# zhaoyuhsin/Edge-Guided-Near-Eye-Image-Analysis-for-Head-Mounted-Displays

Measured on AMD Instinct MI355X. Metric: eye-frames/sec (320x240): inference edge+seg (value), +fit, exact fp32, and train fwd+bwd at 1 MI355X, higher is better.
Workload: dtype f32 tensors; inference products split into f16 hi/lo pairs (3 f16 MFMAs per product, 22-bit significand), f32 accumulate (`exact_fp32`: every product on the f32 MFMA); `train`: bf16 storage, f32 accumulate, f32 master weights (and an f32-storage leg)

## Files before the change

edge-guided-near-eye-image-analysis-for-head-mounted-displays_amd/csrc/common.h:

```cpp
#pragma once
#include <hip/hip_runtime.h>
#include <cstdarg>
#include <cstdio>
#include <mutex>
#include <unordered_map>
#include "../../include/egne_hip.h"

static __device__ __attribute__((aligned(256), used)) float egne_zero_page[64] = {0};

typedef __bf16 egne_bf16;
typedef float egne_f32x4 __attribute__((ext_vector_type(4)));
typedef __bf16 egne_bf16x4 __attribute__((ext_vector_type(4)));
typedef __bf16 egne_bf16x8 __attribute__((ext_vector_type(8)));

__device__ __forceinline__ egne_f32x4 ld4(const float* p) { return *(const egne_f32x4*)p; }
__device__ __forceinline__ egne_f32x4 ld4(const egne_bf16* p) { return __builtin_convertvector(*(const egne_bf16x4*)p, egne_f32x4); }
__device__ __forceinline__ void st4(float* p, egne_f32x4 v) { *(egne_f32x4*)p = v; }
__device__ __forceinline__ void st4(egne_bf16* p, egne_f32x4 v) { *(egne_bf16x4*)p = __builtin_convertvector(v, egne_bf16x4); }
__device__ __forceinline__ float ld1(const float* p) { return *p; }
__device__ __forceinline__ float ld1(const egne_bf16* p) { return (float)*p; }
__device__ __forceinline__ void st1(float* p, float v) { *p = v; }
__device__ __forceinline__ void st1(egne_bf16* p, float v) { *p = (egne_bf16)v; }
template <typename T> struct egne_vt { static constexpr int N = 4; };
template <> struct egne_vt<egne_bf16> { static constexpr int N = 8; };
template <int N> struct egne_fv { float v[N]; };
__device__ __forceinline__ egne_fv<4> ldv(const float* p) {
  const egne_f32x4 t = *(const egne_f32x4*)p;
  return egne_fv<4>{{t[0], t[1], t[2], t[3]}};
}
__device__ __forceinline__ egne_fv<8> ldv(const egne_bf16* p) {
  typedef unsigned u4_ __attribute__((ext_vector_type(4)));
  const u4_ w = *(const u4_*)p;
  egne_fv<8> r;
#pragma unroll
  for (int i = 0; i < 4; ++i) {
    r.v[2 * i] = __builtin_bit_cast(float, w[i] << 16);
    r.v[2 * i + 1] = __builtin_bit_cast(float, w[i] & 0xffff0000u);
  }
  return r;
}
__device__ __forceinline__ void stv(float* p, const egne_fv<4>& a) { *(egne_f32x4*)p = egne_f32x4{a.v[0], a.v[1], a.v[2], a.v[3]}; }
__device__ __forceinline__ void stv(egne_bf16* p, const egne_fv<8>& a) {
  const egne_f32x4 lo = {a.v[0], a.v[1], a.v[2], a.v[3]}, hi = {a.v[4], a.v[5], a.v[6], a.v[7]};
  const egne_bf16x4 l = __builtin_convertvector(lo, egne_bf16x4), h = __builtin_convertvector(hi, egne_bf16x4);
  *(egne_bf16x8*)p = egne_bf16x8{l[0], l[1], l[2], l[3], h[0], h[1], h[2], h[3]};
}
typedef unsigned egne_u32x4 __attribute__((ext_vector_type(4)));
template <typename T> __device__ __forceinline__ egne_u32x4 ldraw(const T* p) { return *(const egne_u32x4*)p; }
__device__ __forceinline__ egne_fv<4> unpackv(const float*, egne_u32x4 w) {
  return egne_fv<4>{{__builtin_bit_cast(float, w[0]), __builtin_bit_cast(float, w[1]), __builtin_bit_cast(float, w[2]), __builtin_bit_cast(float, w[3])}};
}
__device__ __forceinline__ egne_fv<8> unpackv(const egne_bf16*, egne_u32x4 w) {
  egne_fv<8> r;
#pragma unroll
  for (int i = 0; i < 4; ++i) {
    r.v[2 * i] = __builtin_bit_cast(float, w[i] << 16);
    r.v[2 * i + 1] = __builtin_bit_cast(float, w[i] & 0xffff0000u);
  }
  return r;
}
template <int N> __device__ __forceinline__ egne_fv<N> ldf(const float* p) {
  egne_fv<N> r;
#pragma unroll
  for (int i = 0; i < N; i += 4) { const egne_f32x4 t = *(const egne_f32x4*)(p + i); r.v[i] = t[0]; r.v[i + 1] = t[1]; r.v[i + 2] = t[2]; r.v[i + 3] = t[3]; }
  return r;
}
template <int N> __device__ __forceinline__ egne_fv<N> fv_fill(float x) {
  egne_fv<N> r;
#pragma unroll
  for (int i = 0; i < N; ++i) r.v[i] = x;
  return r;
}
template <typename T> __device__ __forceinline__ const T* zero_page() { return (const T*)egne_zero_page; }

#ifdef EGNE_NO_OVF_CHECK
__device__ __forceinline__ bool egne_nonfinite(float) { return false; }
__device__ __forceinline__ bool egne_nonfinite64(double) { return false; }
#else
__device__ __forceinline__ bool egne_nonfinite(float v) { return __builtin_amdgcn_classf(v, 0x207); }
__device__ __forceinline__ bool egne_nonfinite64(double v) { return !__builtin_isfinite(v); }
#endif
__device__ __forceinline__ bool egne_ovf_row(int y, int H) { return y % 3 == 1 || y == H - 1; }
__device__ __forceinline__ void egne_ovf_commit(bool bad, unsigned* flag) {
  if (flag && bad) atomicOr(flag, 1u);
}

namespace egne {

char* err_buf();

inline int fail(int code, const char* fmt, ...) {
  va_list ap;
  va_start(ap, fmt);
  vsnprintf(err_buf(), 512, fmt, ap);
  va_end(ap);
  return code;
}

inline bool fp32_storage(const egne_conv_desc& d) {
  for (int i = 0; i < d.nseg && i < EGNE_MAXSEG; ++i)
    if (d.seg[i].presplit != 0) return false;
  return d.out_split == 0;
}

inline int check_launch(const char* what) {
  hipError_t e = hipGetLastError();
  if (e != hipSuccess) return fail(EGNE_ERR_LAUNCH, "%s: %s", what, hipGetErrorString(e));
  return EGNE_OK;
}

inline bool raise_lds(const void* kern, size_t bytes) {
  static std::mutex mu;
  static std::unordered_map<const void*, size_t> have;
  std::lock_guard<std::mutex> g(mu);
  auto it = have.find(kern);
  if (it != have.end() && it->second >= bytes) return true;
  if (hipFuncSetAttribute(kern, hipFuncAttributeMaxDynamicSharedMemorySize, (int)bytes) != hipSuccess) {
    (void)hipGetLastError();
    return false;
  }
  have[kern] = bytes;
  return true;
}
template <typename... K> inline bool raise_lds_all(size_t bytes, K... kern) { return (raise_lds((const void*)kern, bytes) && ...); }

#define EGNE_REQUIRE(cond, ...) \
  do { if (!(cond)) return ::egne::fail(EGNE_ERR_ARG, __VA_ARGS__); } while (0)

bool halo3_supported(const egne_conv_desc& d);
int halo3_launch(const egne_conv_desc& d, hipStream_t st);

bool wgrad_halo_supported(const egne_conv_desc& d, long long gzs);
int wgrad_halo_splits(const egne_conv_desc& d);
int wgrad_halo_launch(const egne_conv_desc& d, const float* gz, long long gzs, int gzo, float* ws, hipStream_t st);
int wgrad_halo_f16_launch(const egne_conv_desc& d, const float* gz, long long gzs, int gzo, const unsigned* gz_dyn, float* ws, hipStream_t st);

bool wgrad3x3_bf16_supported(const egne_conv_desc& d, long long gzs);
int wgrad3x3_bf16_splits(const egne_conv_desc& d);
int wgrad3x3_bf16_launch(const egne_conv_desc& d, const egne_bf16* gz, long long gzs, int gzo, float* ws, hipStream_t st);
bool wgrad1x1_bf16_supported(const egne_conv_desc& d, long long gzs);
int wgrad1x1_bf16_splits(const egne_conv_desc& d);
int wgrad1x1_bf16_launch(const egne_conv_desc& d, const egne_bf16* gz, long long gzs, int gzo, float* ws, hipStream_t st);

inline int cdiv(long long a, long long b) { return (int)((a + b - 1) / b); }

}
```

edge-guided-near-eye-image-analysis-for-head-mounted-displays_amd/csrc/conv_halo_f16.hip:

```cpp
#include "common.h"
#include "kernel_util.h"
#include "split_f16.h"

namespace {

constexpr int KC = 32, LDH = 40, TW = 32;

__device__ __forceinline__ float act1(float v, int act) {
  if (act == EGNE_ACT_RELU) return fmaxf(v, 0.f);
  if (act == EGNE_ACT_LEAKY) return v > 0.f ? v : 0.01f * v;
  return v;
}


template <int WM, int WN, int D, bool LAT, int NW, int PF = 0, bool TP = false, bool POOL = false, int NP = 3, bool PS = false>
__global__ __launch_bounds__(256, 2) void conv3x3_halo_f16_kernel(const egne_conv_desc p, const _Float16* __restrict__ fhi,
                                                               const _Float16* __restrict__ flo, float a_scale,
                                                               float out_scale, int tiles_x, int tiles_y, int ntiles) {
  egne::dyn_scales(p.dyn_scale, a_scale, out_scale);
  const int vH = TP ? p.W : p.H, vW = TP ? p.H : p.W, rstep = TP ? 1 : p.W, cstep = TP ? p.W : 1;
  constexpr int TH = (4 / NW) * WM;
  constexpr int d = D;
  constexpr int HWd = TW + 2 * d, HHd = TH + 2 * d, npx = HHd * HWd;
  constexpr int nitems = npx * 8;
  constexpr int NI = (nitems + 255) / 256;
  static_assert(HWd >= 32, "one wrap per 32-pixel step");
  static_assert(WN < 3 || (NP == 3 && !PS && !POOL && !LAT && NW == 1), "96-wide tile: three products, fp32 slices, no pooled output");
  extern __shared__ __attribute__((aligned(16))) _Float16 ldsh[];
  _Float16* Ahi = ldsh;
  _Float16* Alo = ldsh + npx * LDH;

  const int tid = threadIdx.x, lane = tid & 63, wave = tid >> 6;
  const int li = lane & 31, lh = lane >> 5;
  const int wrow = wave / NW;
  const int nt0 = (blockIdx.y * NW + wave % NW) * WN;
  const int NT = p.CoutP >> 5, KT16 = p.Ktot >> 4;
  const egne_seg sg = p.seg[0];
  const int Cp = sg.Cp;
  const int c4 = tid & 7;
  const int wave_s = __builtin_amdgcn_readfirstlane(wave);
  auto fresh_tid = [&]() {
    int l;
    asm volatile("v_mbcnt_lo_u32_b32 %0, -1, 0\n\tv_mbcnt_hi_u32_b32 %0, -1, %0" : "=v"(l));
    return wave_s * 64 + l;
  };
  const int S = LAT ? p.dil[0] : 1;
  const unsigned frame_in = (unsigned)p.H * p.W * (unsigned)sg.pix_stride * 4u;
  const unsigned frame_out = (unsigned)p.H * p.W * (unsigned)p.out_pix_stride * 4u;
  const unsigned frame_res = (unsigned)p.H * p.W * (unsigned)p.res_pix_stride * 4u;

  constexpr bool LEAN = WN >= 3;
  int hyx[LEAN ? 1 : NI], roff[LEAN ? 1 : NI];
  if constexpr (!LEAN) {
    int px = tid >> 3;
    int hy = px / HWd, hx = px - hy * HWd;
#pragma unroll
    for (int i = 0; i < NI; ++i) {
      const bool in = tid + 256 * i < nitems;
      hyx[i] = in ? ((S * hy) << 16) | (S * hx) : 0x7fff7fff;
      roff[i] = (S * hy * rstep + S * hx * cstep) * (int)sg.pix_stride * 4 + (PS ? (c4 >> 2) * 64 + (c4 & 3) * 16 : c4 * 16);
      hx += 32;
      if (hx >= HWd) { hx -= HWd; ++hy; }
    }
  }
  const int lofs0 = (tid >> 3) * LDH + c4 * 4;

  struct Tile { int b, y0, x0, py, px; };
  auto tile_of = [&](int t) {
    Tile r;
    const int tx = t % tiles_x; t /= tiles_x;
    const int ty = t % tiles_y; t /= tiles_y;
    r.py = 0; r.px = 0;
    if (LAT) { r.px = t % S; t /= S; r.py = t % S; t /= S; }
    r.b = t; r.y0 = ty * TH; r.x0 = tx * TW;
    return r;
  };

  unsigned goff[NI];
  __amdgpu_buffer_rsrc_t rin = make_rsrc(sg.ptr, 0);
  int stage_b = 0;
  auto map_tile = [&](const Tile& tl) {
    const int ybase = tl.py + S * (tl.y0 - d), xbase = tl.px + S * (tl.x0 - d);
    const int tbase = ((ybase * rstep + xbase * cstep) * (int)sg.pix_stride + sg.ch_off) * 4;
    if constexpr (LEAN) {
      const int tf = fresh_tid();
      const int px = tf >> 3, c4f = tf & 7;
      int hy = px / HWd, hx = px - hy * HWd;
#pragma unroll
      for (int i = 0; i < NI; ++i) {
        const unsigned iy = (unsigned)(ybase + S * hy), ix = (unsigned)(xbase + S * hx);
        const bool in = tf + 256 * i < nitems && iy < (unsigned)vH && ix < (unsigned)vW;
        goff[i] = in ? (unsigned)(tbase + (S * hy * rstep + S * hx * cstep) * (int)sg.pix_stride * 4 + c4f * 16) : OOB;
        hx += 32;
        if (hx >= HWd) { hx -= HWd; ++hy; }
      }
    } else {
#pragma unroll
    for (int i = 0; i < NI; ++i) {
      const unsigned iy = (unsigned)(ybase + (hyx[i] >> 16)), ix = (unsigned)(xbase + (hyx[i] & 0xffff));
      goff[i] = (iy < (unsigned)vH && ix < (unsigned)vW) ? (unsigned)(tbase + roff[i]) : OOB;
    }
    }
    rin = make_rsrc(sg.ptr + (long long)tl.b * p.H * p.W * sg.pix_stride, frame_in);
    stage_b = tl.b;
  };

  u32x4 st[NI];
  f32x4 st_sc = {1.f, 1.f, 1.f, 1.f}, st_sh = {0.f, 0.f, 0.f, 0.f};
  unsigned st_cmask = 0;
  int st_c0 = 0;
  auto load_affine = [&]() {
    const int cq = (LEAN ? fresh_tid() & 7 : c4) * 4;
    const bool cok = st_c0 + cq < Cp;
    st_sc = *(const f32x4*)(cok ? sg.scale + (long long)stage_b * Cp + st_c0 + cq : egne_zero_page);
    st_sh = *(const f32x4*)(cok ? sg.shift + (long long)stage_b * Cp + st_c0 + cq : egne_zero_page);
  };
  auto load_chunk = [&](int c0) {
    const bool cok = PS || c0 + (LEAN ? fresh_tid() & 7 : c4) * 4 < Cp;
    st_cmask = cok ? 0u : OOB;
    st_c0 = c0;
    if (!LEAN && sg.scale) load_affine();
#pragma unroll
    for (int i = 0; i < NI; ++i) st[i] = __builtin_amdgcn_raw_buffer_load_b128(rin, (int)(goff[i] | st_cmask), c0 * 4, 0);
  };
  const float slope_in = sg.act_in == EGNE_ACT_RELU ? 0.f : (sg.act_in == EGNE_ACT_LEAKY ? 0.01f : 1.f);
  const float slope_out = p.act == EGNE_ACT_RELU ? 0.f : (p.act == EGNE_ACT_LEAKY ? 0.01f : 1.f);
  auto store_chunk = [&]() {
    if (sg.scale) {
#pragma unroll
      for (int i = 0; i < NI; ++i) {
        f32x4 v = __builtin_bit_cast(f32x4, st[i]) * st_sc + st_sh;
#pragma unroll
        for (int e = 0; e < 4; ++e) v[e] = fmaxf(v[e], v[e] * slope_in);
        if ((goff[i] | st_cmask) & OOB) v = (f32x4)(0.f);
        st[i] = __builtin_bit_cast(u32x4, v);
      }
    }
    const int tid_s = LEAN ? fresh_tid() : tid;
    const int lofs_s = LEAN ? (tid_s >> 3) * LDH + (tid_s & 7) * 4 : lofs0;
#pragma unroll
    for (int i = 0; i < NI; ++i) {
      if (i < NI - 1 || tid_s + 256 * i < nitems) {
        const f32x4 v = __builtin_bit_cast(f32x4, st[i]);
        const int o = lofs_s + i * 32 * LDH;
        if constexpr (PS) {
          *(u32x4*)&(c4 >> 2 ? Alo : Ahi)[(tid >> 3) * LDH + (c4 & 3) * 8 + i * 32 * LDH] = st[i];
          continue;
        }
        if constexpr (NP == 1) {
          float t0, t1, t2, t3;
          asm("v_mul_f32_e32 %0, %1, %2" : "=v"(t0) : "s"(a_scale), "v"(v[0]));
          asm("v_mul_f32_e32 %0, %1, %2" : "=v"(t1) : "s"(a_scale), "v"(v[1]));
          asm("v_mul_f32_e32 %0, %1, %2" : "=v"(t2) : "s"(a_scale), "v"(v[2]));
          asm("v_mul_f32_e32 %0, %1, %2" : "=v"(t3) : "s"(a_scale), "v"(v[3]));
          const egne::sp_f32x2 u0 = {t0, t1}, u1 = {t2, t3};
          const h2 h0 = __builtin_convertvector(u0, h2), h1 = __builtin_convertvector(u1, h2);
          const h4 hi = {h0[0], h0[1], h1[0], h1[1]};
          *(h4*)&Ahi[o] = hi;
          continue;
        }
        h2 h0, h1, l0, l1;
        egne::split2(v[0], v[1], a_scale, h0, l0);
        egne::split2(v[2], v[3], a_scale, h1, l1);
        const h4 hi = {h0[0], h0[1], h1[0], h1[1]}, lo = {l0[0], l0[1], l1[0], l1[1]};
        *(h4*)&Ahi[o] = hi;
        *(h4*)&Alo[o] = lo;
      }
    }
  };

  f32x16 acc[WM][WN];
#pragma unroll
  for (int a = 0; a < WM; ++a)
#pragma unroll
    for (int n = 0; n < WN; ++n) acc[a][n] = (f32x16)(0.f);

  const unsigned wbytes = 9u * (unsigned)p.Ktot * (unsigned)p.CoutP * 2u;
  const __amdgpu_buffer_rsrc_t rwh = make_rsrc(fhi, wbytes), rwl = make_rsrc(flo, wbytes);
  const int stride_k16 = NT * 1024, stride_tap = KT16 * NT * 1024;
  auto wtap = [&](int t) { return TP ? (t % 3) * 3 + t / 3 : t; };
  const int wlane = lane * 16;

  const int out_step = S * cstep * (int)p.out_pix_stride * 4, res_step = S * cstep * (int)p.res_pix_stride * 4;

  int t = blockIdx.x;
  if (t >= ntiles) return;
  Tile cur = tile_of(t);
  map_tile(cur);
  load_chunk(0);
  int c0 = 0;
  const int abase = (wrow * WM * HWd + li) * LDH + lh * 8;
  while (true) {
    if (LEAN && sg.scale) load_affine();
    __syncthreads();
    store_chunk();
    __syncthreads();
    const bool last_chunk = c0 + KC >= Cp;
    const int tnext = t + gridDim.x;
    auto prefetch = [&]() {
      if (!last_chunk) {
        load_chunk(c0 + KC);
      } else if (tnext < ntiles) {
        const Tile nx = tile_of(tnext);
        map_tile(nx);
        load_chunk(0);
      }
    };
    if (PF == 0) prefetch();
    const int wchunk = nt0 * 1024 + (c0 >> 4) * stride_k16;
    constexpr int RT = (WN == 1 && NW == 1) ? 2 : 1;
    const bool half = Cp - c0 <= 16;
    u32x4 qh[2 * RT][WN], ql[2 * RT][WN];
#pragma unroll
    for (int s = 0; s < 2 * RT; ++s)
#pragma unroll
      for (int tn = 0; tn < WN; ++tn) {
        const int o = wchunk + wtap(s >> 1) * stride_tap + (s & 1) * stride_k16 + tn * 1024;
        const int wl = (half && (s & 1)) ? (int)OOB : wlane;
        qh[s][tn] = __builtin_amdgcn_raw_buffer_load_b128(rwh, wl, o, 0);
        if constexpr (NP == 3) ql[s][tn] = __builtin_amdgcn_raw_buffer_load_b128(rwl, wl, o, 0);
      }
    constexpr int TAP_UNROLL = (NW == 2 || LEAN) ? 1 : 9;
#pragma unroll TAP_UNROLL
    for (int tap = 0; tap < 9; ++tap) {
      const int ky = tap / 3, kx = tap - ky * 3;
      const int aoff = abase + (ky * d * HWd + kx * d) * LDH;
      if (PF == 1 && tap == 1) prefetch();
      if (PF == 2 && tap == 4) prefetch();
#pragma unroll
      for (int ks = 0; ks < 2; ++ks) {
        if (ks == 1 && half) continue;
        const int slot = (tap % RT) * 2 + ks;
        h8 ah[WM], al[WM], bh[WN], bl[WN];
#pragma unroll
        for (int tm = 0; tm < WM; ++tm) {
          ah[tm] = *(const h8*)&Ahi[aoff + tm * HWd * LDH + ks * 16];
          if constexpr (NP == 3) al[tm] = *(const h8*)&Alo[aoff + tm * HWd * LDH + ks * 16];
        }
        if constexpr (LEAN) {
#pragma unroll
          for (int tn = 0; tn < WN; ++tn) {
            const h8 wh = __builtin_bit_cast(h8, qh[slot][tn]), wl_ = __builtin_bit_cast(h8, ql[slot][tn]);
#pragma unroll
            for (int tm = 0; tm < WM; ++tm) {
              acc[tm][tn] = __builtin_amdgcn_mfma_f32_32x32x16_f16(al[tm], wh, acc[tm][tn], 0, 0, 0);
              acc[tm][tn] = __builtin_amdgcn_mfma_f32_32x32x16_f16(ah[tm], wl_, acc[tm][tn], 0, 0, 0);
              acc[tm][tn] = __builtin_amdgcn_mfma_f32_32x32x16_f16(ah[tm], wh, acc[tm][tn], 0, 0, 0);
            }
            if (tap + RT < 9) {
              const int o = wchunk + wtap(tap + RT) * stride_tap + ks * stride_k16 + tn * 1024;
              qh[slot][tn] = __builtin_amdgcn_raw_buffer_load_b128(rwh, wlane, o, 0);
              ql[slot][tn] = __builtin_amdgcn_raw_buffer_load_b128(rwl, wlane, o, 0);
            }
          }
          continue;
        }
#pragma unroll
        for (int tn = 0; tn < WN; ++tn) {
          bh[tn] = __builtin_bit_cast(h8, qh[slot][tn]);
          if constexpr (NP == 3) bl[tn] = __builtin_bit_cast(h8, ql[slot][tn]);
        }
        if (tap + RT < 9) {
#pragma unroll
          for (int tn = 0; tn < WN; ++tn) {
            const int o = wchunk + wtap(tap + RT) * stride_tap + ks * stride_k16 + tn * 1024;
            qh[slot][tn] = __builtin_amdgcn_raw_buffer_load_b128(rwh, wlane, o, 0);
            if constexpr (NP == 3) ql[slot][tn] = __builtin_amdgcn_raw_buffer_load_b128(rwl, wlane, o, 0);
          }
        }
#pragma unroll
        for (int tm = 0; tm < WM; ++tm)
#pragma unroll
          for (int tn = 0; tn < WN; ++tn) {
            if constexpr (NP == 3) {
              acc[tm][tn] = __builtin_amdgcn_mfma_f32_32x32x16_f16(al[tm], bh[tn], acc[tm][tn], 0, 0, 0);
              acc[tm][tn] = __builtin_amdgcn_mfma_f32_32x32x16_f16(ah[tm], bl[tn], acc[tm][tn], 0, 0, 0);
            }
            acc[tm][tn] = __builtin_amdgcn_mfma_f32_32x32x16_f16(ah[tm], bh[tn], acc[tm][tn], 0, 0, 0);
          }
      }
    }
    if (!last_chunk) { c0 += KC; continue; }

    {
      int li_e = li, lh_e = lh, wrow_e = wrow;
      if constexpr (LEAN) {
        const int te = fresh_tid();
        li_e = te & 31; lh_e = (te >> 5) & 1; wrow_e = te >> 6;
      }
      const __amdgpu_buffer_rsrc_t rout = make_rsrc(p.out + (long long)cur.b * p.H * p.W * p.out_pix_stride, frame_out);
      const __amdgpu_buffer_rsrc_t rres =
          make_rsrc(p.residual ? p.residual + (long long)cur.b * p.H * p.W * p.res_pix_stride : nullptr, p.residual ? frame_res : 0u);
      const int xl = cur.px + S * (cur.x0 + 4 * lh_e);
      const int cmax = xl < vW ? (vW - xl + S - 1) / S : 0;
#pragma unroll
      for (int tn = 0; tn < WN; ++tn) {
        const int n = (nt0 + tn) * 32 + li_e;
        const bool nok = n < p.Cout_store;
        const float bv = (p.bias && nok) ? p.bias[n] : 0.f;
        float ps = 1.f, pt = 0.f;
        if (p.post_scale && nok) { ps = p.post_scale[n]; pt = p.post_shift[n]; }
        double st_s = 0., st_q = 0.;
        [[maybe_unused]] float pool_keep[16];
#pragma unroll
        for (int tm = 0; tm < WM; ++tm) {
          const int y = cur.py + S * (cur.y0 + wrow_e * WM + tm);
          const int cm = (nok && y < vH) ? cmax : 0;
          const int pix = y * rstep + xl * cstep;
          const unsigned o0 = (unsigned)((pix * (int)p.out_pix_stride + p.out_ch_off + n) * 4);
          if constexpr (LEAN) {
            const unsigned r0 = (unsigned)((pix * (int)p.res_pix_stride + p.res_ch_off + n) * 4);
#pragma unroll
            for (int rb = 0; rb < 16; rb += 8) {
              float rv[8];
#pragma unroll
              for (int r = 0; r < 8; ++r) {
                const int c = ((rb + r) & 3) + 8 * ((rb + r) >> 2);
                rv[r] = p.residual ? __builtin_bit_cast(float, __builtin_amdgcn_raw_buffer_load_b32(rres, (int)(c < cm ? r0 + c * res_step : OOB), 0, 0)) : 0.f;
              }
#pragma unroll
              for (int r = 0; r < 8; ++r) {
                const int c = ((rb + r) & 3) + 8 * ((rb + r) >> 2);
                float v = acc[tm][tn][rb + r] * out_scale + bv;
                v = fmaxf(v, v * slope_out) * ps + pt + rv[r];
                __builtin_amdgcn_raw_buffer_store_b32(__builtin_bit_cast(unsigned, v), rout, (int)(c < cm ? o0 + c * out_step : OOB), 0, 0);
                const double vm = c < cm ? (double)v : 0.;
                st_s += vm; st_q += vm * vm;
              }
            }
          } else {
          float rv[16];
#pragma unroll
          for (int r = 0; r < 16; ++r) rv[r] = 0.f;
          if (p.residual) {
            const unsigned r0 = (unsigned)((pix * (int)p.res_pix_stride + p.res_ch_off + n) * 4);
#pragma unroll
            for (int r = 0; r < 16; ++r) {
              const int c = (r & 3) + 8 * (r >> 2);
              rv[r] = __builtin_bit_cast(float, __builtin_amdgcn_raw_buffer_load_b32(rres, (int)(c < cm ? r0 + c * res_step : OOB), 0, 0));
            }
          }
#pragma unroll
          for (int r = 0; r < 16; ++r) {
            const int c = (r & 3) + 8 * (r >> 2);
            float v = acc[tm][tn][r] * out_scale + bv;
            v = fmaxf(v, v * slope_out) * ps + pt + rv[r];
            __builtin_amdgcn_raw_buffer_store_b32(__builtin_bit_cast(unsigned, v), rout, (int)(c < cm ? o0 + c * out_step : OOB), 0, 0);
            const double vm = c < cm ? (double)v : 0.;
            st_s += vm; st_q += vm * vm;
            if constexpr (POOL) {
              const float vp = c < cm ? v : -INFINITY;
              if (tm == 0) pool_keep[r] = vp;
              else pool_keep[r] = fmaxf(pool_keep[r], vp);
            }
          }
          }
          acc[tm][tn] = (f32x16)(0.f);
        }
        if constexpr (POOL) {
          if (p.pool_out) {
            const int y = cur.y0 + wrow_e * WM, Hp = (p.H + 1) >> 1, Wp = (p.W + 1) >> 1;
            const __amdgpu_buffer_rsrc_t rpool = make_rsrc(p.pool_out + (long long)cur.b * Hp * Wp * p.pool_pix_stride,
                                                           (unsigned)Hp * Wp * (unsigned)p.pool_pix_stride * 4u);
            const int xl0 = cur.x0 + 4 * lh;
            const unsigned q0 = (unsigned)((((y >> 1) * Wp + (xl0 >> 1)) * (int)p.pool_pix_stride + p.pool_ch_off + n) * 4);
#pragma unroll
            for (int r = 0; r < 16; r += 2) {
              const int c = (r & 3) + 8 * (r >> 2);
              const float m = fmaxf(pool_keep[r], pool_keep[r + 1]);
              const bool ok = nok && y < p.H && xl0 + c < p.W;
              __builtin_amdgcn_raw_buffer_store_b32(__builtin_bit_cast(unsigned, m), rpool, (int)(ok ? q0 + (c >> 1) * (int)p.pool_pix_stride * 4 : OOB), 0, 0);
            }
          }
        }
        if (!LAT && NW == 1 && p.stats_ws) {
          st_s += __shfl_xor(st_s, 32); st_q += __shfl_xor(st_q, 32);
          if (lh_e == 0 && n < p.Cout_store) {
            const int tile_in_frame = (cur.y0 / TH) * tiles_x + cur.x0 / TW;
            double2* w = (double2*)p.stats_ws + ((long long)cur.b * p.stats_nchunk + tile_in_frame * 4 + wrow_e) * p.Cout_store + n;
            *w = make_double2(st_s, st_q);
          }
        }
      }
    }
    t = tnext;
    if (t >= ntiles) break;
    cur = tile_of(t);
    c0 = 0;
  }
}

__global__ void pack_weight_f16frag_k(const float* __restrict__ w, int Cout, int Cin, int T, int CoutP, int Ktot, float wscale,
                                      _Float16* __restrict__ hi, _Float16* __restrict__ lo) {
  const long long total = (long long)T * CoutP * Ktot;
  const int NT = CoutP >> 5;
  for (long long i = (long long)blockIdx.x * blockDim.x + threadIdx.x; i < total; i += (long long)gridDim.x * blockDim.x) {
    const int j = (int)(i & 7), nn = (int)((i >> 3) & 31), h = (int)((i >> 8) & 1);
    long long q = i >> 9;
    const int nt = (int)(q % NT); q /= NT;
    const int k16 = (int)(q % (Ktot >> 4));
    const int t = (int)(q / (Ktot >> 4));
    const int n = nt * 32 + nn, k = k16 * 16 + h * 8 + j;
    const float v = (n < Cout && k < Cin) ? w[((long long)n * Cin + k) * T + t] * wscale : 0.f;
    const _Float16 hh = (_Float16)v;
    hi[i] = hh;
    lo[i] = (_Float16)(v - (float)hh);
  }
}

template <int WM, int WN, int D, bool LAT, int NW = 1, int PF = 0, bool TP = false, int NP = 3, bool PS = false>
int launch_hf_tp(const egne_conv_desc& d, const _Float16* fhi, const _Float16* flo, float a_scale, float os, hipStream_t st) {
  constexpr int TH = (4 / NW) * WM;
  const int S = LAT ? d.dil[0] : 1;
  const int vH = TP ? d.W : d.H, vW = TP ? d.H : d.W;
  const int lw = (vW + S - 1) / S, lh_ = (vH + S - 1) / S;
  const int tiles_x = (lw + TW - 1) / TW, tiles_y = (lh_ + TH - 1) / TH;
  const size_t lds = (size_t)2 * (TH + 2 * D) * (TW + 2 * D) * LDH * sizeof(_Float16);
  const int ntiles = tiles_x * tiles_y * d.B * S * S, ny = d.CoutP / (32 * WN * NW);
  int gx = (256 * 2 + ny - 1) / ny;
  if (gx > ntiles) gx = ntiles;
  hipLaunchKernelGGL((conv3x3_halo_f16_kernel<WM, WN, D, LAT, NW, PF, TP, false, NP, PS>), dim3(gx, ny), dim3(256), lds, st, d, fhi, flo, a_scale, os, tiles_x,
                     tiles_y, ntiles);
  return egne::check_launch("egne_conv3x3_halo_f16_fwd");
}

template <int WM, int WN, int D, bool LAT, int NW = 1, int PF = 0, int NP = 3, bool PS = false>
int launch_hf(const egne_conv_desc& d, const _Float16* fhi, const _Float16* flo, float a_scale, float os, hipStream_t st) {
  constexpr int TH = (4 / NW) * WM;
  const int S = LAT ? d.dil[0] : 1;
  auto ntile = [&](int vh, int vw) { return ((((vw + S - 1) / S) + TW - 1) / TW) * ((((vh + S - 1) / S) + TH - 1) / TH); };
  static const bool tall_ok = [] { const char* e = getenv("EGNE_SHALO_TALL"); return !e || e[0] != '0'; }();
  if (D == 1 && NW == 1 && PF == 0 && tall_ok && ntile(d.W, d.H) < ntile(d.H, d.W))
    return launch_hf_tp<WM, WN, (D == 1 && NW == 1 && PF == 0 ? D : 1), LAT, (D == 1 && NW == 1 && PF == 0 ? NW : 1), 0, true, NP, PS>(d, fhi, flo, a_scale, os, st);
  return launch_hf_tp<WM, WN, D, LAT, NW, PF, false, NP, PS>(d, fhi, flo, a_scale, os, st);
}

}

extern "C" int egne_pack_conv_weight_f16frag(const float* w_oihw, int Cout, int Cin, int kh, int kw, int CoutP, int Ktot,
                                             float wscale, void* fhi, void* flo, void* stream) {
  EGNE_REQUIRE(w_oihw && fhi && flo && Cout > 0 && Cin > 0 && CoutP >= Cout && CoutP % 32 == 0 && Ktot >= Cin && Ktot % 32 == 0,
               "pack_f16frag: bad sizes Cout %d Cin %d CoutP %d Ktot %d", Cout, Cin, CoutP, Ktot);
  long long total = (long long)kh * kw * CoutP * Ktot, g = (total + 255) / 256;
  if (g > 4096) g = 4096;
  hipLaunchKernelGGL(pack_weight_f16frag_k, dim3((unsigned)g), dim3(256), 0, (hipStream_t)stream, w_oihw, Cout, Cin, kh * kw, CoutP,
                     Ktot, wscale, (_Float16*)fhi, (_Float16*)flo);
  return egne::check_launch("egne_pack_conv_weight_f16frag");
}

extern "C" int egne_conv3x3_halo_f16_fwd(const egne_conv_desc* dp, const void* fhi, const void* flo, float a_scale,
                                         float w_scale, void* stream) {
  EGNE_REQUIRE(dp && fhi && flo, "conv_halo_f16: null pointer");
  const egne_conv_desc& d = *dp;
  EGNE_REQUIRE(d.kh == 3 && d.kw == 3 && d.stride == 1 && d.pad_mode == 0 && d.ngroups == 1 && d.nseg == 1 && d.pad_h == 1 &&
               d.pad_w == 1 && d.dil[0] >= 1 && d.dil[0] <= 32 && d.Ho == d.H && d.Wo == d.W, "conv_halo_f16: geometry not supported");
  const egne_seg& g = d.seg[0];
  EGNE_REQUIRE(g.ptr && g.Cp % 8 == 0 && (g.Cp + 31) / 32 * 32 == d.Ktot && g.ch_off % 4 == 0 && g.pix_stride % 4 == 0 &&
               ((uintptr_t)g.ptr & 15) == 0 && (g.scale == nullptr) == (g.shift == nullptr), "conv_halo_f16: input slice");
  EGNE_REQUIRE(d.CoutP % 32 == 0 && d.Cout_store <= d.CoutP && d.out && d.out_ch_off + d.Cout_store <= d.out_pix_stride,
               "conv_halo_f16: CoutP %d", d.CoutP);
  EGNE_REQUIRE(((uintptr_t)fhi & 15) == 0 && ((uintptr_t)flo & 15) == 0 && a_scale > 0.f && w_scale > 0.f, "conv_halo_f16: weights / scales");
  {
    const int t_n = ((d.W + 31) / 32) * ((d.H + 7) / 8), t_t = ((d.H + 31) / 32) * ((d.W + 7) / 8);
    static const bool tall_on = [] { const char* e = getenv("EGNE_SHALO_TALL"); return !e || e[0] != '0'; }();
    const int tiles = (tall_on && t_t < t_n) ? t_t : t_n;
    EGNE_REQUIRE(!d.stats_ws || (d.dil[0] == 1 && ((uintptr_t)d.stats_ws & 15) == 0 && d.stats_nchunk == tiles * 4),
                 "conv_halo_f16: stats_ws needs dilation 1 and stats_nchunk = tiles * 4 (%d tiles per frame)", tiles);
  }
  EGNE_REQUIRE((long long)d.H * d.W * g.pix_stride * 4 < (1ll << 31) && (long long)d.H * d.W * d.out_pix_stride * 4 < (1ll << 31) &&
               (!d.residual || (long long)d.H * d.W * d.res_pix_stride * 4 < (1ll << 31)), "conv_halo_f16: frame too large for 32-bit byte offsets");
  const float os = 1.0f / (a_scale * w_scale);
  hipStream_t st = (hipStream_t)stream;
  const _Float16* h = (const _Float16*)fhi;
  const _Float16* l = (const _Float16*)flo;
  EGNE_REQUIRE(g.presplit == 0 || (g.presplit == 3 && d.dil[0] == 1 && d.CoutP == 32 && !g.scale && !d.dyn_scale && d.f16_products != 1 && !d.pool_out &&
                                   g.Cp % 32 == 0 && g.ch_off % 32 == 0),
               "conv_halo_f16: presplit %d: 0, or 3 on a raw slice of whole 32-channel blocks (dilation 1, CoutP 32, three products)", g.presplit);
  if (g.presplit == 3) return launch_hf<2, 1, 1, false, 1, 0, 3, true>(d, (const _Float16*)fhi, (const _Float16*)flo, a_scale, os, st);
  const bool w2 = d.CoutP % 64 == 0;
  const bool w3 = d.CoutP == 96 && d.dil[0] == 1 && d.f16_products != 1 && !d.pool_out;
  static const int nw2 = [] { const char* e = getenv("EGNE_SHALO_NW2"); return e ? atoi(e) : 0; }();
  if (nw2 && w2) {
    if (d.dil[0] == 1) return launch_hf<4, 1, 1, false, 2>(d, h, l, a_scale, os, st);
    if (d.dil[0] == 2) return launch_hf<4, 1, 2, false, 2>(d, h, l, a_scale, os, st);
    return launch_hf<4, 1, 1, true, 2>(d, h, l, a_scale, os, st);
  }
  if (d.pool_out) {
    EGNE_REQUIRE(d.dil[0] == 1 && !d.post_scale && !d.residual && !d.stats_ws && ((uintptr_t)d.pool_out & 3) == 0 &&
                 d.pool_ch_off + d.Cout_store <= d.pool_pix_stride &&
                 (long long)((d.H + 1) / 2) * ((d.W + 1) / 2) * d.pool_pix_stride * 4 < (1ll << 31), "conv_halo_f16: pooled second output");
    constexpr size_t lds = (size_t)2 * (8 + 2) * (TW + 2) * LDH * sizeof(_Float16);
    const int tiles_x = (d.W + TW - 1) / TW, tiles_y = (d.H + 7) / 8, ntiles = tiles_x * tiles_y * d.B;
    const int ny = d.CoutP / (w2 ? 64 : 32);
    int gx = (256 * 2 + ny - 1) / ny;
    if (gx > ntiles) gx = ntiles;
    if (w2 && d.f16_products == 1) hipLaunchKernelGGL((conv3x3_halo_f16_kernel<2, 2, 1, false, 1, 0, false, true, 1>), dim3(gx, ny), dim3(256), lds, st, d, h, l, a_scale, os, tiles_x, tiles_y, ntiles);
    else if (w2) hipLaunchKernelGGL((conv3x3_halo_f16_kernel<2, 2, 1, false, 1, 0, false, true>), dim3(gx, ny), dim3(256), lds, st, d, h, l, a_scale, os, tiles_x, tiles_y, ntiles);
    else hipLaunchKernelGGL((conv3x3_halo_f16_kernel<2, 1, 1, false, 1, 0, false, true>), dim3(gx, ny), dim3(256), lds, st, d, h, l, a_scale, os, tiles_x, tiles_y, ntiles);
    return egne::check_launch("egne_conv3x3_halo_f16_fwd");
  }
  static const int pf = [] { const char* e = getenv("EGNE_SHALO_PF"); return e ? atoi(e) : 0; }();
  if (d.dil[0] == 1 && pf == 1) return w2 ? launch_hf<2, 2, 1, false, 1, 1>(d, h, l, a_scale, os, st) : launch_hf<2, 1, 1, false, 1, 1>(d, h, l, a_scale, os, st);
  if (d.dil[0] == 1 && pf == 2) return w2 ? launch_hf<2, 2, 1, false, 1, 2>(d, h, l, a_scale, os, st) : launch_hf<2, 1, 1, false, 1, 2>(d, h, l, a_scale, os, st);
  if (d.dil[0] == 1 && d.f16_products == 1) return w2 ? launch_hf<2, 2, 1, false, 1, 0, 1>(d, h, l, a_scale, os, st) : launch_hf<2, 1, 1, false, 1, 0, 1>(d, h, l, a_scale, os, st);
  if (w3) return launch_hf<2, 3, 1, false>(d, h, l, a_scale, os, st);
  if (d.dil[0] == 1) return w2 ? launch_hf<2, 2, 1, false>(d, h, l, a_scale, os, st) : launch_hf<2, 1, 1, false>(d, h, l, a_scale, os, st);
  if (d.dil[0] == 2) return w2 ? launch_hf<2, 2, 2, false>(d, h, l, a_scale, os, st) : launch_hf<2, 1, 2, false>(d, h, l, a_scale, os, st);
  return w2 ? launch_hf<2, 2, 1, true>(d, h, l, a_scale, os, st) : launch_hf<2, 1, 1, true>(d, h, l, a_scale, os, st);
}
```

Baseline: 2206.

## Stream halo conv weights through a double-buffered LDS ring via buffer-to-LDS DMA

Adds a WL variant of the 3x3 halo f16 conv kernel for dilation-1, three-product shapes. Weight fragments are DMA'd from global memory straight into a two-slot LDS ring, so they no longer go through registers, and the next group's copy overlaps the MFMA work on the current group. This path is on by default for the plain and pooled launches. It costs extra LDS per workgroup, which may lower occupancy, and adds more barriers per chunk. The change also includes optional timestamp instrumentation, a probe script, and a per-device key for the LDS-raise cache.

```diff
diff --git a/edge-guided-near-eye-image-analysis-for-head-mounted-displays_amd/csrc/common.h b/edge-guided-near-eye-image-analysis-for-head-mounted-displays_amd/csrc/common.h
--- a/edge-guided-near-eye-image-analysis-for-head-mounted-displays_amd/csrc/common.h
+++ b/edge-guided-near-eye-image-analysis-for-head-mounted-displays_amd/csrc/common.h
@@ -2,8 +2,10 @@
 #include <hip/hip_runtime.h>
 #include <cstdarg>
 #include <cstdio>
+#include <map>
 #include <mutex>
 #include <unordered_map>
+#include <utility>
 #include "../../include/egne_hip.h"
 
 static __device__ __attribute__((aligned(256), used)) float egne_zero_page[64] = {0};
@@ -111,15 +113,21 @@
 
 inline bool raise_lds(const void* kern, size_t bytes) {
   static std::mutex mu;
-  static std::unordered_map<const void*, size_t> have;
+  static std::map<std::pair<int, const void*>, size_t> have;
+  int dev = 0;
+  if (hipGetDevice(&dev) != hipSuccess) {
+    (void)hipGetLastError();
+    return false;
+  }
   std::lock_guard<std::mutex> g(mu);
-  auto it = have.find(kern);
+  const auto key = std::make_pair(dev, kern);
+  auto it = have.find(key);
   if (it != have.end() && it->second >= bytes) return true;
   if (hipFuncSetAttribute(kern, hipFuncAttributeMaxDynamicSharedMemorySize, (int)bytes) != hipSuccess) {
     (void)hipGetLastError();
     return false;
   }
-  have[kern] = bytes;
+  have[key] = bytes;
   return true;
 }
 template <typename... K> inline bool raise_lds_all(size_t bytes, K... kern) { return (raise_lds((const void*)kern, bytes) && ...); }
diff --git a/edge-guided-near-eye-image-analysis-for-head-mounted-displays_amd/csrc/conv_halo_f16.hip b/edge-guided-near-eye-image-analysis-for-head-mounted-displays_amd/csrc/conv_halo_f16.hip
--- a/edge-guided-near-eye-image-analysis-for-head-mounted-displays_amd/csrc/conv_halo_f16.hip
+++ b/edge-guided-near-eye-image-analysis-for-head-mounted-displays_amd/csrc/conv_halo_f16.hip
@@ -1,6 +1,23 @@
 #include "common.h"
 #include "kernel_util.h"
 #include "split_f16.h"
+
+#ifdef EGNE_HALO_STAMPS
+__device__ unsigned long long egne_halo_stamps_buf[1024 * 4 * 8];
+extern "C" int egne_halo_read_stamps(unsigned long long* host) {
+  return hipMemcpyFromSymbol(host, HIP_SYMBOL(egne_halo_stamps_buf), sizeof(egne_halo_stamps_buf)) == hipSuccess ? 0 : 1;
+}
+#define HS_T0() unsigned long long hs_last = __builtin_amdgcn_s_memtime(), hs_acc[6] = {0, 0, 0, 0, 0, 0}; const unsigned long long hs_begin = hs_last
+#define HS_ADD(i) do { const unsigned long long hs_now = __builtin_amdgcn_s_memtime(); hs_acc[i] += hs_now - hs_last; hs_last = hs_now; } while (0)
+#define HS_CHUNK() do { hs_acc[5] += 1; } while (0)
+#define HS_OUT() do { if (lane == 0) { unsigned long long* o = egne_halo_stamps_buf + (((blockIdx.y * gridDim.x + blockIdx.x) & 1023) * 4 + wave) * 8; \
+  for (int i = 0; i < 6; ++i) o[i] = hs_acc[i]; o[6] = __builtin_amdgcn_s_memtime() - hs_begin; } } while (0)
+#else
+#define HS_T0() do {} while (0)
+#define HS_ADD(i) do {} while (0)
+#define HS_CHUNK() do {} while (0)
+#define HS_OUT() do {} while (0)
+#endif
 
 namespace {
 
@@ -13,7 +30,7 @@
 }
 
 
-template <int WM, int WN, int D, bool LAT, int NW, int PF = 0, bool TP = false, bool POOL = false, int NP = 3, bool PS = false>
+template <int WM, int WN, int D, bool LAT, int NW, int PF = 0, bool TP = false, bool POOL = false, int NP = 3, bool PS = false, bool WL = false>
 __global__ __launch_bounds__(256, 2) void conv3x3_halo_f16_kernel(const egne_conv_desc p, const _Float16* __restrict__ fhi,
                                                                const _Float16* __restrict__ flo, float a_scale,
                                                                float out_scale, int tiles_x, int tiles_y, int ntiles) {
@@ -29,6 +46,9 @@
   extern __shared__ __attribute__((aligned(16))) _Float16 ldsh[];
   _Float16* Ahi = ldsh;
   _Float16* Alo = ldsh + npx * LDH;
+  static_assert(!WL || (D == 1 && !LAT && NW == 1 && NP == 3 && PF == 0 && 6 % WN == 0), "weights through LDS: the dilation-1 three-product shapes");
+  constexpr int WSLOT = 12 * 1024, GS = 6 / WN, NG = 18 / GS;
+  char* const wring = (char*)(ldsh + 2 * npx * LDH);
 
   const int tid = threadIdx.x, lane = tid & 63, wave = tid >> 6;
   const int li = lane & 31, lh = lane >> 5;
@@ -180,6 +200,16 @@
   const int stride_k16 = NT * 1024, stride_tap = KT16 * NT * 1024;
   auto wtap = [&](int t) { return TP ? (t % 3) * 3 + t / 3 : t; };
   const int wlane = lane * 16;
+  auto dma_group = [&](int g, int slot, int wch) {
+#pragma unroll
+    for (int i = 0; i < 3; ++i) {
+      const int j = 4 * i + wave_s, r = (12 * g + j) >> 1;
+      const int tn = r % WN, sk = r / WN;
+      const int o = wch + wtap(sk >> 1) * stride_tap + (sk & 1) * stride_k16 + tn * 1024;
+      __builtin_amdgcn_raw_ptr_buffer_load_lds((wave_s & 1) ? rwl : rwh, (lds_ptr)(wring + slot * WSLOT + j * 1024), 16, wlane, o, 0, 0);
+    }
+  };
+  int wslot = 0;
 
   const int out_step = S * cstep * (int)p.out_pix_stride * 4, res_step = S * cstep * (int)p.res_pix_stride * 4;
 
@@ -189,12 +219,25 @@
   map_tile(cur);
   load_chunk(0);
   int c0 = 0;
+  if constexpr (WL) dma_group(0, 0, nt0 * 1024);
   const int abase = (wrow * WM * HWd + li) * LDH + lh * 8;
+  HS_T0();
   while (true) {
     if (LEAN && sg.scale) load_affine();
+    HS_ADD(4);
+    if constexpr (WL) {
+      asm volatile("s_waitcnt vmcnt(0)" ::: "memory");
+      lds_barrier();
+      dma_group(1, wslot ^ 1, nt0 * 1024 + (c0 >> 4) * stride_k16);
+      store_chunk();
+      lds_barrier();
+    } else {
     __syncthreads();
     store_chunk();
     __syncthreads();
+    }
+    HS_ADD(0);
+    HS_CHUNK();
     const bool last_chunk = c0 + KC >= Cp;
     const int tnext = t + gridDim.x;
     auto prefetch = [&]() {
@@ -206,10 +249,79 @@
         load_chunk(0);
       }
     };
-    if (PF == 0) prefetch();
+    if (PF == 0 && !WL) prefetch();
     const int wchunk = nt0 * 1024 + (c0 >> 4) * stride_k16;
     constexpr int RT = (WN == 1 && NW == 1) ? 2 : 1;
     const bool half = Cp - c0 <= 16;
+    if constexpr (WL) {
+      const bool more = !last_chunk || tnext < ntiles;
+      const bool pf_first = !LEAN && sg.scale != nullptr;
+      const int wnext = nt0 * 1024 + (last_chunk ? 0 : ((c0 + KC) >> 4) * stride_k16);
+      constexpr int TAP_UNROLL_W = LEAN ? 1 : 9;
+#pragma unroll TAP_UNROLL_W
+      for (int tap = 0; tap < 9; ++tap) {
+        const int ky = tap / 3, kx = tap - ky * 3;
+        const int aoff = abase + (ky * d * HWd + kx * d) * LDH;
+#pragma unroll
+        for (int ks = 0; ks < 2; ++ks) {
+          const int step = tap * 2 + ks;
+          if (step % GS == 0 && step > 0) {
+            const int g = step / GS;
+            HS_ADD(1);
+            if (g == 2 && more && !pf_first) asm volatile("s_waitcnt vmcnt(%0)" :: "n"(NI) : "memory");
+            else asm volatile("s_waitcnt vmcnt(0)" ::: "memory");
+            HS_ADD(2);
+            lds_barrier();
+            HS_ADD(3);
+            wslot ^= 1;
+            if (g == 1 && pf_first) prefetch();
+            if (g + 1 < NG) dma_group(g + 1, wslot ^ 1, wchunk);
+            else if (more) dma_group(0, wslot ^ 1, wnext);
+            if (g == 1 && !pf_first) {
+              asm volatile("" ::: "memory");
+              __builtin_amdgcn_sched_barrier(0);
+              prefetch();
+            }
+          }
+          if (ks == 1 && half) continue;
+          const char* wf = wring + wslot * WSLOT + (step % GS) * (WN * 2048) + wlane;
+          h8 ah[WM], al[WM];
+#pragma unroll
+          for (int tm = 0; tm < WM; ++tm) {
+            ah[tm] = *(const h8*)&Ahi[aoff + tm * HWd * LDH + ks * 16];
+            al[tm] = *(const h8*)&Alo[aoff + tm * HWd * LDH + ks * 16];
+          }
+          if constexpr (LEAN) {
+#pragma unroll
+            for (int tn = 0; tn < WN; ++tn) {
+              const h8 wh = *(const h8*)(wf + tn * 2048), wl_ = *(const h8*)(wf + tn * 2048 + 1024);
+#pragma unroll
+              for (int tm = 0; tm < WM; ++tm) {
+                acc[tm][tn] = __builtin_amdgcn_mfma_f32_32x32x16_f16(al[tm], wh, acc[tm][tn], 0, 0, 0);
+                acc[tm][tn] = __builtin_amdgcn_mfma_f32_32x32x16_f16(ah[tm], wl_, acc[tm][tn], 0, 0, 0);
+                acc[tm][tn] = __builtin_amdgcn_mfma_f32_32x32x16_f16(ah[tm], wh, acc[tm][tn], 0, 0, 0);
+              }
+            }
+          } else {
+            h8 bh[WN], bl[WN];
+#pragma unroll
+            for (int tn = 0; tn < WN; ++tn) {
+              bh[tn] = *(const h8*)(wf + tn * 2048);
+              bl[tn] = *(const h8*)(wf + tn * 2048 + 1024);
+            }
+#pragma unroll
+            for (int tm = 0; tm < WM; ++tm)
+#pragma unroll
+              for (int tn = 0; tn < WN; ++tn) {
+                acc[tm][tn] = __builtin_amdgcn_mfma_f32_32x32x16_f16(al[tm], bh[tn], acc[tm][tn], 0, 0, 0);
+                acc[tm][tn] = __builtin_amdgcn_mfma_f32_32x32x16_f16(ah[tm], bl[tn], acc[tm][tn], 0, 0, 0);
+                acc[tm][tn] = __builtin_amdgcn_mfma_f32_32x32x16_f16(ah[tm], bh[tn], acc[tm][tn], 0, 0, 0);
+              }
+          }
+        }
+      }
+      wslot ^= 1;
+    } else {
     u32x4 qh[2 * RT][WN], ql[2 * RT][WN];
 #pragma unroll
     for (int s = 0; s < 2 * RT; ++s)
@@ -280,6 +392,8 @@
           }
       }
     }
+    }
+    HS_ADD(1);
     if (!last_chunk) { c0 += KC; continue; }
 
     {
@@ -388,6 +502,7 @@
     cur = tile_of(t);
     c0 = 0;
   }
+  HS_OUT();
 }
 
 __global__ void pack_weight_f16frag_k(const float* __restrict__ w, int Cout, int Cin, int T, int CoutP, int Ktot, float wscale,
@@ -408,6 +523,13 @@
   }
 }
 
+template <int WM, int D, bool LAT, int NW, int PF, int NP> constexpr bool wlds_build = WM == 2 && D == 1 && !LAT && NW == 1 && PF == 0 && NP == 3;
+constexpr size_t WLDS_RING = 2 * 12 * 1024;
+inline bool wlds_on() {
+  const char* e = getenv("EGNE_SHALO_WLDS");
+  return !(e && e[0] == '0');
+}
+
 template <int WM, int WN, int D, bool LAT, int NW = 1, int PF = 0, bool TP = false, int NP = 3, bool PS = false>
 int launch_hf_tp(const egne_conv_desc& d, const _Float16* fhi, const _Float16* flo, float a_scale, float os, hipStream_t st) {
   constexpr int TH = (4 / NW) * WM;
@@ -419,6 +541,14 @@
   const int ntiles = tiles_x * tiles_y * d.B * S * S, ny = d.CoutP / (32 * WN * NW);
   int gx = (256 * 2 + ny - 1) / ny;
   if (gx > ntiles) gx = ntiles;
+  if constexpr (wlds_build<WM, D, LAT, NW, PF, NP>) {
+    if (wlds_on()) {
+      auto kern = conv3x3_halo_f16_kernel<WM, WN, D, LAT, NW, PF, TP, false, NP, PS, true>;
+      if (!egne::raise_lds((const void*)kern, lds + WLDS_RING)) return egne::fail(EGNE_ERR_LAUNCH, "conv_halo_f16: cannot raise the dynamic LDS limit to %zu", lds + WLDS_RING);
+      hipLaunchKernelGGL(kern, dim3(gx, ny), dim3(256), lds + WLDS_RING, st, d, fhi, flo, a_scale, os, tiles_x, tiles_y, ntiles);
+      return egne::check_launch("egne_conv3x3_halo_f16_fwd");
+    }
+  }
   hipLaunchKernelGGL((conv3x3_halo_f16_kernel<WM, WN, D, LAT, NW, PF, TP, false, NP, PS>), dim3(gx, ny), dim3(256), lds, st, d, fhi, flo, a_scale, os, tiles_x,
                      tiles_y, ntiles);
   return egne::check_launch("egne_conv3x3_halo_f16_fwd");
@@ -494,6 +624,13 @@
     const int ny = d.CoutP / (w2 ? 64 : 32);
     int gx = (256 * 2 + ny - 1) / ny;
     if (gx > ntiles) gx = ntiles;
+    if (d.f16_products != 1 && wlds_on()) {
+      auto k2 = conv3x3_halo_f16_kernel<2, 2, 1, false, 1, 0, false, true, 3, false, true>;
+      auto k1 = conv3x3_halo_f16_kernel<2, 1, 1, false, 1, 0, false, true, 3, false, true>;
+      if (!egne::raise_lds_all(lds + WLDS_RING, k2, k1)) return egne::fail(EGNE_ERR_LAUNCH, "conv_halo_f16: cannot raise the dynamic LDS limit to %zu", lds + WLDS_RING);
+      hipLaunchKernelGGL(w2 ? k2 : k1, dim3(gx, ny), dim3(256), lds + WLDS_RING, st, d, h, l, a_scale, os, tiles_x, tiles_y, ntiles);
+      return egne::check_launch("egne_conv3x3_halo_f16_fwd");
+    }
     if (w2 && d.f16_products == 1) hipLaunchKernelGGL((conv3x3_halo_f16_kernel<2, 2, 1, false, 1, 0, false, true, 1>), dim3(gx, ny), dim3(256), lds, st, d, h, l, a_scale, os, tiles_x, tiles_y, ntiles);
     else if (w2) hipLaunchKernelGGL((conv3x3_halo_f16_kernel<2, 2, 1, false, 1, 0, false, true>), dim3(gx, ny), dim3(256), lds, st, d, h, l, a_scale, os, tiles_x, tiles_y, ntiles);
     else hipLaunchKernelGGL((conv3x3_halo_f16_kernel<2, 1, 1, false, 1, 0, false, true>), dim3(gx, ny), dim3(256), lds, st, d, h, l, a_scale, os, tiles_x, tiles_y, ntiles);
diff --git a/scratch/halo_wlds_stamps.py b/scratch/halo_wlds_stamps.py
--- /dev/null
+++ b/scratch/halo_wlds_stamps.py
@@ -0,0 +1,38 @@
+import ctypes as C, os, sys
+ROOT = os.path.dirname(os.path.dirname(os.path.abspath(__file__)))
+sys.path.insert(0, ROOT); sys.path.insert(0, os.path.join(ROOT, 'tests'))
+import numpy as np, torch
+import egne_amd
+from egne_amd import _lib
+import test_gpu_halo_wlds as T
+T.B = int(sys.argv[1]) if len(sys.argv) > 1 else 64
+L = _lib.lib()
+L.egne_halo_read_stamps.restype = C.c_int; L.egne_halo_read_stamps.argtypes = [C.c_void_p]
+
+
+class Env:
+    def setenv(self, k, v):
+        os.environ[k] = v
+
+
+CASES = [("vgg.conv2_2  <2,2> pooled", T._case("s1", 120, 160, 128, 128, act=T.RELU, pool=True)),
+         ("enc.b1.conv1 <2,2> affine", T._case("s2", 120, 160, 76, 64, norm=True, stats=True)),
+         ("enc.b2       <2,3> affine", T._case("s3", 60, 80, 100, 96, norm=True, stats=True)),
+         ("dec.up3      <2,2> affine", T._case("s4", 60, 80, 64, 64, norm=True)),
+         ("ms3 split-pair <2,1>", T._case("s5", 60, 80, 256, 32, act=T.RELU, ps=True)),
+         ("ms4 split-pair <2,1>", T._case("s6", 30, 40, 256, 32, act=T.RELU, ps=True))]
+T.CASES.extend(c for _, c in CASES)
+for name, case in CASES:
+    d = T._data(case)
+    for form in (False, True):
+        T._launch(L, case, d, form, Env())
+        torch.cuda.synchronize()
+        buf = np.zeros(1024 * 4 * 8, dtype=np.uint64)
+        L.egne_halo_read_stamps(buf.ctypes.data_as(C.c_void_p))
+        ny = max(1, T._pad(case["Cout"], 32) // (96 if case["Cout"] == 96 else 64))
+        nwg = min((512 + ny - 1) // ny, T._tiles(case["H"], case["W"]) * T.B) * ny
+        st = buf.reshape(1024, 4, 8).astype(np.float64)[:nwg]
+        ch = st[:, :, 5]
+        per = lambda i: (st[:, :, i] / ch).mean()
+        print("%-28s %-13s workgroups %4d chunks/wave %5.1f | cycles per chunk: staging %6.0f  MFMA issue %6.0f  ring wait %5.0f  hand-over barriers %5.0f  epilogue + tile change %6.0f | total %6.0f" % (
+            name, "LDS ring" if form else "register ring", nwg, ch.mean(), per(0), per(1), per(2), per(3), per(4), (st[:, :, 6] / ch).mean()), flush=True)
```

Result: no change. 2215 (median of 6 runs) (+0.4%).
